# epruesse/metacov

Hardware: AMD Instinct MI355X
Metric: aligned bases/sec into per-position depth vector, 1/2/4/8 MI355X (higher is better)
Workload: dtype int32

## Files before the change

### metacov_amd/csrc/engine.hip

```cpp
#include <hip/hip_ext.h>
#include <hip/hip_runtime.h>

#include <algorithm>
#include <atomic>
#include <cmath>
#include <cstdlib>
#include <cstring>
#include <vector>

#include "../../include/metacov_amd.h"
#include "common.h"
#include "kernels.h"
#include "npstd.h"
#include "capmask.h"

#include <hipcub/hipcub.hpp>

using namespace mc;

#ifndef MC_PLAIN_TILES_PER_CHUNK
#define MC_PLAIN_TILES_PER_CHUNK 4
#endif
constexpr int kPlainTilesPerChunk = MC_PLAIN_TILES_PER_CHUNK;

// ... 1169 lines not shown
    const bool lds_hist = nbins <= kLdsBins;
    HIP_TRY(hipEventRecord(ctx->ev[6], s));
    int64_t launches = 0;
    for (int64_t r0 = 0; r0 < R; r0 += rb) {
        const int64_t nr = std::min(rb, R - r0);
        std::vector<int64_t> sg_gs, sg_ge, ntot(nr), nzx(nr);
        std::vector<int32_t> sg_reg;
        int64_t covered = 0;
        for (int64_t k = 0; k < nr; ++k) {
            const int64_t ext = ctx->extent[tid[r0 + k]];
            covered += std::min(end[r0 + k], ext) - std::min(start[r0 + k], ext);
        }
        int64_t seg = kSeg;
        while (seg > 16384 && covered / seg < 2048) seg >>= 1;
        for (int64_t k = 0; k < nr; ++k) {
            const int64_t r = r0 + k;
            const int32_t t = tid[r];
            const int64_t ext = ctx->extent[t];
            const int64_t a = std::min(start[r], ext), b = std::min(end[r], ext);
            ntot[k] = end[r] - start[r];
            nzx[k] = ntot[k] - (b - a);
            for (int64_t p = a; p < b; p += seg) {
                sg_gs.push_back(ctx->coff[t] + p);
                sg_ge.push_back(ctx->coff[t] + std::min(b, p + seg));
                sg_reg.push_back((int32_t)k);
            }
        }
        const int64_t nseg = (int64_t)sg_gs.size();
        const size_t o_gs = 0, o_ge = o_gs + stage_align(nseg * 8),
                     o_reg = o_ge + stage_align(nseg * 8), o_ntot = o_reg + stage_align(nseg * 4),
                     o_nzx = o_ntot + stage_align(nr * 8), o_rows = o_nzx + stage_align(nr * 8),
                     total = o_rows + (out_rows ? stage_align(nr * 8) : 0);
        HIP_TRY(ctx->k3_stage.reserve(total));
        unsigned char* h = ctx->k3_stage.host();
        std::memcpy(h + o_gs, sg_gs.data(), nseg * 8);
        std::memcpy(h + o_ge, sg_ge.data(), nseg * 8);
        std::memcpy(h + o_reg, sg_reg.data(), nseg * 4);
        std::memcpy(h + o_ntot, ntot.data(), nr * 8);
        std::memcpy(h + o_nzx, nzx.data(), nr * 8);
        if (out_rows) std::memcpy(h + o_rows, out_rows + r0, nr * 8);
        unsigned char* d = ctx->k3_stage.d.p;
        const int64_t* d_seg_gs = reinterpret_cast<const int64_t*>(d + o_gs);
        const int64_t* d_seg_ge = reinterpret_cast<const int64_t*>(d + o_ge);
        const int32_t* d_seg_reg = reinterpret_cast<const int32_t*>(d + o_reg);
        HIP_TRY(ctx->d_hist.reserve((size_t)round_up(nr * nbins, 4)));
        HIP_TRY(ctx->d_acc.reserve(nr));
        HIP_TRY(hipMemcpyAsync(d, h, total, hipMemcpyHostToDevice, s));
        {
            const int64_t hw = round_up(nr * nbins, 4);
            const int64_t work = std::max<int64_t>(hw / 4, nr);
            const unsigned g = (unsigned)std::min<int64_t>(4096, (work + kBlock - 1) / kBlock);
            hipLaunchKernelGGL(fused_init_kernel, dim3(std::max(g, 1u)), dim3(kBlock), 0, s,
                               ctx->d_hist.p, hw, (unsigned*)nullptr, ctx->d_acc.p, nr,
                               (const int64_t*)nullptr, (int64_t)0, (int64_t)1, (int64_t)0,
                               (int64_t*)nullptr, (unsigned*)nullptr, (int*)nullptr);
            HIP_TRY(hipGetLastError());
        }
        if (nseg) {
            if (lds_hist)
                hipLaunchKernelGGL(region_seg_kernel<true>, dim3((unsigned)nseg), dim3(kBlock),
                                   (size_t)round_up(nbins, 4) * 4, s, ctx->d_depth.p, d_seg_gs, d_seg_ge,
                                   d_seg_reg, nbins, ctx->d_hist.p, ctx->d_acc.p);
            else
                hipLaunchKernelGGL(region_seg_kernel<false>, dim3((unsigned)nseg), dim3(kBlock), 0,
                                   s, ctx->d_depth.p, d_seg_gs, d_seg_ge, d_seg_reg, nbins,
                                   ctx->d_hist.p, ctx->d_acc.p);
            HIP_TRY(hipGetLastError());
            ++launches;
        }
        hipLaunchKernelGGL(region_final_kernel, dim3((unsigned)nr), dim3(kBlock), 0, s,
                           ctx->d_hist.p, nbins, ctx->d_acc.p,
                           reinterpret_cast<const int64_t*>(d + o_ntot),
                           reinterpret_cast<const int64_t*>(d + o_nzx),
                           out_rows ? d_out_final : d_out_final + r0, (int*)nullptr, 1,
                           (const int32_t*)nullptr, (const unsigned*)nullptr, 1,
                           out_rows ? reinterpret_cast<const int64_t*>(d + o_rows) : nullptr);
        HIP_TRY(hipGetLastError());
        HIP_TRY(hipStreamSynchronize(s));
    }
    HIP_TRY(hipEventRecord(ctx->ev[7], s));
    ctx->t_stats = true;
    ctx->t.stats_launches += launches;
    return MC_OK;
}


struct FusedLayout {
    size_t gs, ge, id, base, ntot, nzx, brow, rtid, rfused, up, total;
};
static FusedLayout fused_layout(int64_t nf, int64_t R) {
    auto al = stage_align;
    FusedLayout L;
    L.gs = 0;
    L.ge = L.gs + al(nf * 8);
    L.id = L.ge + al(nf * 8);
    L.base = L.id + al(nf * 4);
    L.ntot = L.base + al(nf * 4);
    L.nzx = L.ntot + al(R * 8);
    L.brow = L.nzx + al(R * 8);
    L.rtid = L.brow + al(R * 4);
    L.rfused = L.rtid + al(R * 4);
    L.up = L.rfused + al(R * 4);
    L.total = L.up;
    return L;
}

constexpr int kRedo = 1;

static size_t fflag_ints(int64_t R) { return (size_t)round_up(R + 1, 2) + 2 * kDresWords; }
static unsigned long long* fflag_dres(int* base, int64_t R) {
    return reinterpret_cast<unsigned long long*>(base + round_up(R + 1, 2));
}

static int direct_verdict_sync(mc_ctx* ctx) {
    if (!ctx->direct || ctx->direct_checked) return MC_OK;
    unsigned long long* res = static_cast<unsigned long long*>(ctx->pin_io.h);
    HIP_TRY(hipMemcpyAsync(res, ctx->d_dres.p, kDresWords * 8, hipMemcpyDeviceToHost, ctx->stream));
    HIP_TRY(hipStreamSynchronize(ctx->stream));
    if (check_direct(ctx, res)) return MC_OK;
    direct_fallback(ctx, res);
    return kRedo;
}

#ifndef MC_DONE_MODE
#define MC_DONE_MODE 1
#endif
static int wait_event_spin(hipEvent_t ev) {
    for (;;) {
        const hipError_t e = hipEventQuery(ev);
        if (e == hipSuccess) return MC_OK;
        if (e != hipErrorNotReady) HIP_TRY(e);
        __builtin_ia32_pause();
    }
}

static int wait_stamp(mc_ctx* ctx, unsigned long long seq) {
    if (!ctx->stamp_ok) {
        HIP_TRY(hipStreamSynchronize(ctx->stream));
        return MC_OK;
    }
    for (unsigned k = 1;; ++k) {
        if (__atomic_load_n(ctx->h_done.h, __ATOMIC_ACQUIRE) >= seq) return MC_OK;
        __builtin_ia32_pause();
        if ((k & 1023) == 0) {
            const hipError_t e = hipStreamQuery(ctx->stream);
            if (e == hipSuccess) return MC_OK;
            if (e != hipErrorNotReady) HIP_TRY(e);
        }
    }
}

static int depth_stats_launch(mc_ctx* ctx, int64_t R, const int32_t* tid, const int64_t* start,
                              const int64_t* end, RegionOut* d_out, int64_t nf) {
    hipStream_t s = ctx->stream;
    const FusedLayout L = fused_layout(nf, R);
    const size_t o_gs = L.gs, o_ge = L.ge, o_id = L.id, o_base = L.base, o_ntot = L.ntot,
                 o_nzx = L.nzx, o_brow = L.brow;
    const K2Geom geo = k2_geom(ctx, true);
    HIP_TRY(ctx->d_fchunk.reserve(geo.n_chunks));
    HIP_TRY(ctx->d_flow.reserve(R));
    const int vals = fused_hist_vals(ctx->has_long);
    HIP_TRY(ctx->d_fhist.reserve((size_t)(R * vals)));
    HIP_TRY(ctx->h_fflag.reserve(fflag_ints(R)));
    const bool verdict = ctx->direct && !ctx->direct_checked;
    HIP_TRY(ctx->d_acc.reserve(R));
    unsigned char* d = ctx->fstage.d.p;
    const int64_t* d_fge = reinterpret_cast<const int64_t*>(d + o_ge);
    const bool clean = ctx->fused_clean && ctx->fused_clean_R == R && ctx->fcache.chunk_first;
    ctx->fused_clean = false;
    if (!clean) {
        const int64_t idx_chunks = ctx->fcache.chunk_first ? 0 : geo.n_chunks;
        const int64_t work = std::max<int64_t>({R * vals / 4, R, idx_chunks});
        const unsigned g = (unsigned)std::min<int64_t>(4096, (work + kBlock - 1) / kBlock);
        hipLaunchKernelGGL(fused_init_kernel, dim3(std::max(g, 1u)), dim3(kBlock), 0, s,
                           ctx->d_fhist.p, R * vals, ctx->d_flow.p, ctx->d_acc.p, R, d_fge, nf,
                           geo.chunk_w, idx_chunks, ctx->d_fchunk.p, ctx->d_queue.p,
                           ctx->d_maxdepth.p);
        HIP_TRY(hipGetLastError());
        ctx->fcache.chunk_first = true;
    } else if (ctx->check_clean) {
        HIP_TRY(ctx->d_check.reserve(1));
        HIP_TRY(hipMemsetAsync(ctx->d_check.p, 0, sizeof(unsigned long long), s));
        hipLaunchKernelGGL(fused_clean_check_kernel, dim3(1024), dim3(kBlock), 0, s, ctx->d_fhist.p, R * vals,
                           ctx->d_flow.p, ctx->d_acc.p, R, ctx->d_queue.p, ctx->d_maxdepth.p, ctx->d_check.p);
        HIP_TRY(hipGetLastError());
        unsigned long long bad = 0;
        HIP_TRY(hipMemcpyAsync(&bad, ctx->d_check.p, sizeof bad, hipMemcpyDeviceToHost, s));
        HIP_TRY(hipStreamSynchronize(s));
        MC_REQUIRE(bad == 0, MC_E_STATE, "fused buffers not initialised on a clean call (%llu words differ)", bad);
    }
    FusedRegions fr{nf,
                    ctx->d_fchunk.p,
                    reinterpret_cast<const int64_t*>(d + o_gs),
                    d_fge,
                    reinterpret_cast<const int32_t*>(d + o_id),
                    reinterpret_cast<const int32_t*>(d + o_base),
                    reinterpret_cast<const int32_t*>(d + L.rtid),
                    ctx->d_acc.p,
                    ctx->d_fhist.p,
                    ctx->d_flow.p};
    if (nf == 0) fr.n = 0;
    auto& T = ctx->ts[ctx->ts_cur];
    if (int rc = launch_depth(ctx, fr, T.e[1], T.e[2])) return rc;
    const unsigned long long seq = ++ctx->done_seq;
    unsigned long long* stamp = nullptr;
    if (ctx->stamp_ok) {
        if (!ctx->h_done.h) {
            if (ctx->h_done.reserve(1) != hipSuccess || ctx->d_kdone.reserve(1) != hipSuccess ||
                hipMemsetAsync(ctx->d_kdone.p, 0, sizeof(unsigned), s) != hipSuccess) {
                (void)hipGetLastError();
                ctx->stamp_ok = false;
            } else {
                __atomic_store_n(ctx->h_done.h, 0ull, __ATOMIC_RELEASE);
            }
        }
        if (ctx->stamp_ok && MC_DONE_MODE == 1) stamp = ctx->h_done.d;
    }
    const bool devfb = ctx->has_long || ctx->fb_recent;
    FbArgs F{};
    if (devfb) {
        if (!ctx->d_fb_cnt.p) {
            HIP_TRY(ctx->d_fb_hist.reserve((size_t)kFbSlots * kLdsBins));
            HIP_TRY(ctx->d_fb_acc.reserve(kFbSlots));
            HIP_TRY(ctx->d_fb_list.reserve(kFbSlots));
            HIP_TRY(ctx->d_fb_cnt.reserve(2));
            HIP_TRY(hipMemsetAsync(ctx->d_fb_cnt.p, 0, 8, s));
            hipLaunchKernelGGL(fused_init_kernel, dim3(1024), dim3(kBlock), 0, s, ctx->d_fb_hist.p,
                               (int64_t)kFbSlots * kLdsBins, (unsigned*)nullptr, ctx->d_fb_acc.p,
                               (int64_t)kFbSlots, (const int64_t*)nullptr, (int64_t)0, (int64_t)1, (int64_t)0,
                               (int64_t*)nullptr, (unsigned*)nullptr, (int*)nullptr);
            HIP_TRY(hipGetLastError());
        }
        F = FbArgs{ctx->d_depth.p,
                   reinterpret_cast<const int32_t*>(d + L.rfused),
                   reinterpret_cast<const int64_t*>(d + o_gs),
                   reinterpret_cast<const int64_t*>(d + o_ge),
                   reinterpret_cast<const int64_t*>(d + o_ntot),
                   reinterpret_cast<const int64_t*>(d + o_nzx),
                   ctx->h_fflag.d + R,
                   ctx->d_fb_list.p,
                   ctx->d_fb_cnt.p,
                   (int)(ctx->fb_calls & 1),
                   ctx->d_fb_hist.p,
                   ctx->d_fb_acc.p,
                   d_out};
        ctx->fb_calls += 1;
    }
    hipEvent_t k3_stop = MC_STEP_EVENTS && MC_EXT_EVENTS ? T.e[3] : nullptr;
#define MC_LAUNCH_K3B(V)                                                                           \
    hipExtLaunchKernelGGL(region_final_wave_kernel<V>, dim3((unsigned)((R + kWaves - 1) / kWaves)),     \
                          dim3(kBlock), 0u, s, nullptr, devfb ? nullptr : k3_stop, 0u,                   \
                          ctx->d_fhist.p, R, ctx->d_acc.p,                                              \
                       reinterpret_cast<const int64_t*>(d + o_ntot),                                \
                       reinterpret_cast<const int64_t*>(d + o_nzx), d_out, ctx->h_fflag.d,           \
                       reinterpret_cast<const int32_t*>(d + o_brow), ctx->d_flow.p,                 \
                       ctx->d_maxdepth.p, ctx->h_fflag.d + R, ctx->d_queue.p,                       \
                       verdict ? ctx->d_dres.p : nullptr, verdict ? fflag_dres(ctx->h_fflag.d, R) : nullptr, \
                       devfb ? F.cnt + F.parity : nullptr, devfb ? F.list : nullptr,                \
                       ctx->direct ? direct_window(ctx) : DirectWindow{},                          \
                       ctx->direct ? reinterpret_cast<const int32_t*>(d + L.rtid) : nullptr,           \
                       ctx->d_kdone.p, devfb ? nullptr : stamp, seq)
    if (vals == HistCfg<false>::kBins) MC_LAUNCH_K3B(HistCfg<false>::kBins);
    else MC_LAUNCH_K3B(HistCfg<true>::kBins);
#undef MC_LAUNCH_K3B
    HIP_TRY(hipGetLastError());
    if (devfb) {
        hipLaunchKernelGGL(fb_seg_kernel, dim3(1024), dim3(kBlock), (size_t)kLdsBins * 4, s, F);
        HIP_TRY(hipGetLastError());
        hipExtLaunchKernelGGL(fb_final_kernel, dim3(kFbSlots), dim3(kBlock), 0u, s, nullptr, k3_stop, 0u, F);
        HIP_TRY(hipGetLastError());
    }
    if (MC_STEP_EVENTS && !MC_EXT_EVENTS) HIP_TRY(hipEventRecord(T.e[3], s));
    if ((MC_DONE_MODE == 0 || (MC_DONE_MODE == 1 && devfb)) && ctx->stamp_ok && hipStreamWriteValue64(s, ctx->h_done.d, seq, 0) != hipSuccess) {
        (void)hipGetLastError();
        ctx->stamp_ok = false;
    }
    ctx->t_stats = false;
    ctx->t.stats_launches += 1;
    resolve_timings(ctx, false);
    if (int rc = MC_DONE_MODE == 2 ? wait_event_spin(T.e[3]) : wait_stamp(ctx, seq)) return rc;
    const int* flags = ctx->h_fflag.h;
    if (verdict && !check_direct(ctx, fflag_dres(ctx->h_fflag.h, R), true)) {
// ... 467 lines not shown
```

### metacov_amd/csrc/kernels.h

```cpp
#pragma once

#include <hip/hip_runtime.h>
#include <stdint.h>

namespace mc {

#ifndef MC_TILE_W
#define MC_TILE_W 4096
#endif
#ifndef MC_RING
#define MC_RING (2 * MC_TILE_W)
#endif
#ifndef MC_TILES_PER_CHUNK
#define MC_TILES_PER_CHUNK 8
#endif
#ifndef MC_PREFETCH
#define MC_PREFETCH 1
#endif
#ifndef MC_PREFETCH_STATS
#define MC_PREFETCH_STATS 1
#endif
#ifndef MC_APPLY_SHORT
#define MC_APPLY_SHORT 1
#endif
#ifndef MC_FAR_HALO
#define MC_FAR_HALO 1
#endif
#ifndef MC_FAR_HALO_MIN
#define MC_FAR_HALO_MIN 4096
#endif
#ifndef MC_DIRECT_ONE_CONTIG
#define MC_DIRECT_ONE_CONTIG 1
#endif
#ifndef MC_K2_WAVE_ADVANCE
#define MC_K2_WAVE_ADVANCE 0
#endif
#ifndef MC_FILL_WAVE_COUNTS
#define MC_FILL_WAVE_COUNTS 0
#endif
#ifndef MC_FILL_SORTED
#define MC_FILL_SORTED 0
#endif
#ifndef MC_DEFER_LONG
#define MC_DEFER_LONG 1
#endif
#ifndef MC_DEFER_DIRECT
#define MC_DEFER_DIRECT 0
#endif
#ifndef MC_NT_STORE
#define MC_NT_STORE 1
#endif
#ifndef MC_WAVES_PLAIN
#define MC_WAVES_PLAIN 0
#endif
#ifndef MC_WAVES_STATS
#define MC_WAVES_STATS 4
#endif
constexpr int kGposBits = 18;
constexpr unsigned kGposMask = (1u << kGposBits) - 1u;
constexpr int kGspanCap = (1 << (32 - kGposBits)) - 1;

constexpr int kBlock = 256;
constexpr int kWaves = kBlock / 64;
constexpr int kTileW = MC_TILE_W;
constexpr int kRing = MC_RING;
static_assert(kRing % 256 == 0 && kRing > kTileW, "ring must hold a tile plus a halo");

__device__ __forceinline__ int ring_slot(int rel) { return rel % kRing; }
constexpr int kTilesPerChunk = MC_TILES_PER_CHUNK;
#ifndef MC_TILES_PER_CHUNK_LONG
#define MC_TILES_PER_CHUNK_LONG 16
#endif
constexpr int kTilesPerChunkLong = MC_TILES_PER_CHUNK_LONG;
constexpr int kReadsPerThread = 4;
constexpr int kBatch = kBlock * kReadsPerThread;
#ifndef MC_K2_WAVES
#define MC_K2_WAVES 4
#endif
constexpr int kK2Waves = MC_K2_WAVES;
constexpr int kK2Block = 64 * kK2Waves;
constexpr int kK2Batch = kK2Block * kReadsPerThread;
constexpr int kPadBatch = kK2Batch > kBatch ? kK2Batch : kBatch;
static_assert(kK2Waves == 4 || kK2Waves == 8, "K2 workgroups of 4 or 8 waves");
constexpr int kLdsHeader = (4 + 2 * kK2Waves + 4 + 3) / 4 * 4 > 20 ? (4 + 2 * kK2Waves + 4 + 3) / 4 * 4 : 20;
constexpr int kSeg = 65536;
constexpr int kLdsBins = 16384;

typedef int i32x4 __attribute__((ext_vector_type(4)));

struct RegionAcc {
    unsigned long long sum;
    unsigned long long sumsq;
    int min;
    int max;
};


__device__ __forceinline__ int wave_incl_scan(int v, int lane) {
    (void)lane;
    v += __builtin_amdgcn_update_dpp(0, v, 0x111, 0xf, 0xf, false);
    v += __builtin_amdgcn_update_dpp(0, v, 0x112, 0xf, 0xf, false);
    v += __builtin_amdgcn_update_dpp(0, v, 0x114, 0xf, 0xf, false);
    v += __builtin_amdgcn_update_dpp(0, v, 0x118, 0xf, 0xf, false);
    v += __builtin_amdgcn_update_dpp(0, v, 0x142, 0xa, 0xf, false);
    v += __builtin_amdgcn_update_dpp(0, v, 0x143, 0xc, 0xf, false);
    return v;
}

__device__ __forceinline__ int wave_sum_i32(int v) {
// ... 421 lines not shown
#pragma unroll
        for (int w = 1; w < kWaves; ++w)
            v = threadIdx.x == 3 ? max(v, red[3][w]) : v + red[threadIdx.x][w];
        if (threadIdx.x == 3) atomicMax(&out[3], (unsigned long long)v);
        else if (v) atomicAdd(&out[threadIdx.x], (unsigned long long)v);
    }
}

constexpr int kProbeShift = 8;
constexpr int kNearHalo = 256;
constexpr int kFarHaloMin = MC_FAR_HALO_MIN;
constexpr int kProbeStride = 1 << kProbeShift;

enum : int {
    kDresBadSample = 0,
    kDresLongSample = 1,
    kDresFlags = 2,
    kDresBases = 3,
    kDresMaxSpan = 4,
    kDresSpanSum = 5,
    kDresSpanCnt = 6,
    kDresWords = 9
};
constexpr unsigned kDirectInvalid = 1;
constexpr unsigned kDirectUnfit = 2;

struct ProbeArgs {
    const int32_t* tid;
    const int32_t* pos;
    const int32_t* span;
    int64_t n;
    int32_t nc;
    const int64_t* coff;
    int lw;
    int short_max;
    int halo;
    int64_t n_base;
    int32_t* j0;
    int32_t* jh;
    int32_t* jn;
    int32_t* fsamp;
    unsigned long long* dres;
    unsigned long long gen;
};

struct DirectWindow {
    const int32_t* fsamp;
    const int64_t* len;
    const unsigned long long* dres;
    int parity;
    int win_below;
};

template <class WT>
__device__ __forceinline__ int direct_window_base(const WT& W, int parity, int t) {
    const long long ns = (long long)uload(W.fsamp, t + 1) - uload(W.fsamp, t);
    const unsigned long long ssum = uload(W.dres, kDresSpanSum + 2 * parity);
    const unsigned long long scnt = uload(W.dres, kDresSpanCnt + 2 * parity);
    if (ns <= 0 || scnt == 0) return 0;
    const double mean = (double)ssum / (double)scnt;
    const double bases = (double)ns * (double)kProbeStride * mean;
    const double ext = (double)uload(W.len, t);
    const double body = ext > 2.0 * mean ? ext - mean : ext;
    const double est = ext > 0 ? bases / body : 0.0;
    const long long b0 = llrint(est) - W.win_below;
    return b0 > 0 ? (int)b0 : 0;
}

__device__ __forceinline__ int64_t probe_key(const ProbeArgs& A, int t, int p) {
    const int ct = t < 0 ? 0 : t >= A.nc ? A.nc - 1 : t;
    const int64_t k = A.coff[ct] + (int64_t)(p < 0 ? 0 : p);
    return k;
}

__device__ __forceinline__ void probe_fill(int32_t* J, int64_t n_base, int lw, int64_t off, int64_t key,
                                           int64_t key_next, bool first, bool last, int32_t val) {
    int64_t k0 = first ? 0 : ((key + off) >> lw) + 1;
    int64_t k1 = last ? n_base : ((key_next + off) >> lw);
    if (k1 > n_base) k1 = n_base;
    if (first) {
        int64_t kz = (key + off) >> lw;
        if (kz > n_base) kz = n_base;
        for (int64_t k = 0; k <= kz; ++k) J[k] = 0;
        k0 = kz + 1;
    }
    for (int64_t k = k0; k <= k1; ++k) J[k] = val;
}

constexpr int kProbeSpanEvery = 4;
constexpr unsigned kProbeMeanBlocks = 64;

__global__ void __launch_bounds__(kBlock)
probe_kernel(ProbeArgs A) {
    const int64_t M = (A.n + kProbeStride - 1) >> kProbeShift;
    const int64_t j = (int64_t)blockIdx.x * kBlock + threadIdx.x;
    const int par = (int)(A.gen & 1);
    if (blockIdx.x == 0 && threadIdx.x >= kDresFlags && threadIdx.x <= kDresMaxSpan) A.dres[threadIdx.x] = 0;
    if (blockIdx.x == 0 && threadIdx.x < 2) A.dres[kDresSpanSum + 2 * (par ^ 1) + threadIdx.x] = 0;
    const bool sampled = j < M && (j % kProbeSpanEvery) == 0;
    const int s0 = sampled ? A.span[j << kProbeShift] : 0;
    const unsigned every = max(1u, gridDim.x / kProbeMeanBlocks);
    if (blockIdx.x % every == 0) {
        __shared__ long long red[2 * kWaves];
        const bool s_ok = sampled && s0 >= 0;
        const long long wsum = wave_sum64(s_ok ? (long long)s0 : 0);
        const long long wcnt = wave_sum64(s_ok ? 1 : 0);
        if ((threadIdx.x & 63) == 0) {
            red[threadIdx.x >> 6] = wsum;
            red[kWaves + (threadIdx.x >> 6)] = wcnt;
        }
        __syncthreads();
        if (threadIdx.x == 0) {
            long long ts = 0, tc = 0;
#pragma unroll
            for (int w = 0; w < kWaves; ++w) {
                ts += red[w];
                tc += red[kWaves + w];
            }
            if (tc) {
// ... 832 lines not shown
    __syncthreads();
    if (threadIdx.x == 0) {
        long long t = 0;
#pragma unroll
        for (int w = 0; w < kWaves; ++w) t += ws[w];
        part[blockIdx.x] = (unsigned long long)t;
    }
}

__global__ void __launch_bounds__(kBlock)
span_sum_final_kernel(const unsigned long long* __restrict__ part, int m, unsigned long long* __restrict__ out) {
    long long s = 0;
    for (int i = threadIdx.x; i < m; i += kBlock) s += (long long)part[i];
    s = wave_sum64(s);
    __shared__ long long ws[kWaves];
    if ((threadIdx.x & 63) == 0) ws[threadIdx.x >> 6] = s;
    __syncthreads();
    if (threadIdx.x == 0) {
        long long t = 0;
#pragma unroll
        for (int w = 0; w < kWaves; ++w) t += ws[w];
        *out = (unsigned long long)t;
    }
}

#ifndef MC_HIST_COPIES
#define MC_HIST_COPIES 2
#endif
#ifndef MC_HIST_BINS
#define MC_HIST_BINS (MC_HIST_COPIES == 1 ? 1024 : MC_HIST_COPIES == 2 ? 864 \
                      : MC_HIST_COPIES == 4 ? 480 : MC_HIST_COPIES == 8 ? 224 : 96)
#endif
#ifndef MC_HIST_COPIES_LONG
#define MC_HIST_COPIES_LONG MC_HIST_COPIES
#endif
#ifndef MC_HIST_BINS_LONG
#define MC_HIST_BINS_LONG (MC_HIST_COPIES_LONG == 1 ? 1728 : MC_HIST_BINS)
#endif
template <bool kLong>
struct HistCfg {
    static constexpr int kCopies = kLong ? MC_HIST_COPIES_LONG : MC_HIST_COPIES;
    static constexpr int kBins = kLong ? MC_HIST_BINS_LONG : MC_HIST_BINS;
    static constexpr int kPad = kCopies > 1 ? 32 / kCopies : 32;
    static constexpr int kStride = kBins + kPad;
    static constexpr int kLds = kCopies * kStride;
    static_assert(kBins % 32 == 0 && (kCopies & (kCopies - 1)) == 0 && kCopies <= 32,
                  "histogram bins: multiple of 32; copies: power of two");
};
constexpr int kHistBins = HistCfg<false>::kBins;
__host__ __device__ constexpr int fused_hist_vals(bool long_reads) {
    return long_reads ? HistCfg<true>::kBins : HistCfg<false>::kBins;
}

struct FusedRegions {
    int64_t n;
    const int64_t* chunk_first;
    const int64_t* gs;
    const int64_t* ge;
    const int32_t* id;
    const int32_t* base;
    const int32_t* rtid;
    RegionAcc* acc;
    unsigned* hist;
    unsigned* low;
};

struct OvLds {
    unsigned long long sum, sq;
    int vmin, vmax;
    unsigned cnt, low;
    unsigned pad[2];
};
constexpr int kOvRecs = 16;
static_assert(sizeof(OvLds) == 40, "record stride: 10 banks");
constexpr int kOvInts = kOvRecs * (int)sizeof(OvLds) / 4;

__device__ __forceinline__ void ov_reset(OvLds* ov) {
    ov->sum = ov->sq = 0;
    ov->vmin = 0x7fffffff;
    ov->vmax = 0;
    ov->cnt = ov->low = 0;
}

struct OvReg {
    unsigned cnt, low;
    unsigned long long sum, sq;
    int vmin, vmax;
};

__device__ __forceinline__ void ov_reg_reset(OvReg& r) {
    r.cnt = r.low = 0;
    r.sum = r.sq = 0;
    r.vmin = 0x7fffffff;
    r.vmax = 0;
}

__device__ __attribute__((noinline)) void ov_spill(OvLds* ov, unsigned cnt, unsigned low, unsigned long long sum,
                                                   unsigned long long sq, int mn, int mx) {
    if (cnt) {
        atomicAdd(&ov->cnt, cnt);
        if (low) atomicAdd(&ov->low, low);
        atomicAdd(&ov->sum, sum);
        atomicAdd(&ov->sq, sq);
        atomicMin(&ov->vmin, mn);
        atomicMax(&ov->vmax, mx);
    }
}

__device__ __forceinline__ void ov_reg_spill(OvReg& r, OvLds* ovf) {
    if (__any(r.cnt != 0)) {
        ov_spill(ovf + (threadIdx.x & (kOvRecs - 1)), r.cnt, r.low, r.sum, r.sq, r.vmin, r.vmax);
        ov_reg_reset(r);
    }
}

static_assert(kRing == 2 * kTileW, "the ring tail is one tile (short_max = kTileW)");

template <int kWinBins>
__device__ __forceinline__ void hist_int4(unsigned* h, int dummy, OvReg& ovr, int y0, int y1, int y2, int y3,
                                          int base) {
    const bool s1 = y1 != y0, s2 = y2 != y1, s3 = y3 != y2;
    const int l2 = s3 ? 1 : 2;
    const int l1 = s2 ? 1 : l2 + 1;
    const int l0 = s1 ? 1 : l1 + 1;
    constexpr unsigned kWin = (unsigned)kWinBins;
    const unsigned du = (unsigned)dummy;
    const unsigned d0 = (unsigned)(y0 - base), d1 = (unsigned)(y1 - base),
                   d2 = (unsigned)(y2 - base), d3 = (unsigned)(y3 - base);
    atomicAdd(&h[min(d0, du)], (unsigned)l0);
    atomicAdd(&h[s1 ? min(d1, du) : du], (unsigned)l1);
    atomicAdd(&h[s2 ? min(d2, du) : du], (unsigned)l2);
    atomicAdd(&h[s3 ? min(d3, du) : du], 1u);
    if (__builtin_expect(__any(max(max(d0, d1), max(d2, d3)) >= kWin), 0)) {
        const int y[4] = {y0, y1, y2, y3};
        const unsigned d[4] = {d0, d1, d2, d3};
#pragma unroll
        for (int k = 0; k < 4; ++k) {
            const bool o = (y[k] >= 0) & (d[k] >= kWin);
            const unsigned v = o ? (unsigned)y[k] : 0u;
            ovr.cnt += o ? 1u : 0u;
            ovr.low += (o & (y[k] < base)) ? 1u : 0u;
            ovr.sum += v;
            ovr.sq += (unsigned long long)v * v;
            ovr.vmin = min(ovr.vmin, o ? y[k] : 0x7fffffff);
            ovr.vmax = max(ovr.vmax, (int)v);
        }
    }
}

__device__ __forceinline__ void block_all2(int* words, int& flip, bool p0, bool p1, int wave, int lane,
                                           bool& all0, bool& all1) {
    const int v = (__all(p0) ? 1 : 0) | (__all(p1) ? 2 : 0);
    if (lane == 0) reinterpret_cast<unsigned char*>(words + 2 * flip)[wave] = (unsigned char)v;
    __syncthreads();
    if (kK2Waves == 4) {
        const int w = words[2 * flip];
        all0 = (w & 0x01010101) == 0x01010101;
        all1 = (w & 0x02020202) == 0x02020202;
    } else {
        const unsigned long long w = *reinterpret_cast<const unsigned long long*>(words + 2 * flip);
        all0 = (w & 0x0101010101010101ull) == 0x0101010101010101ull;
        all1 = (w & 0x0202020202020202ull) == 0x0202020202020202ull;
    }
    flip ^= 1;
}

struct EvBatch {
    int rel[4];
    unsigned pending;
};

__device__ __forceinline__ void load_events(EvBatch& e, const int32_t* __restrict__ ev, int64_t base,
                                            int64_t e_lo, int64_t e_hi) {
    const int64_t i0 = base + (int64_t)threadIdx.x * 4;
    e.pending = 0;
    if (i0 < e_hi && i0 + 4 > e_lo) {
        const i32x4 x = *reinterpret_cast<const i32x4*>(ev + i0);
        e.rel[0] = x.x;
        e.rel[1] = x.y;
        e.rel[2] = x.z;
        e.rel[3] = x.w;
#pragma unroll
        for (int k = 0; k < 4; ++k)
            if (i0 + k >= e_lo && i0 + k < e_hi) e.pending |= 1u << k;
    }
}

template <bool kBarriers, class HC, class RT>
__device__ __forceinline__ void flush_region(const RT& R, int id, unsigned* h, OvLds* ov) {
    if (kBarriers) __syncthreads();
    if (threadIdx.x < kOvRecs) {
        OvLds* o = ov + threadIdx.x;
        if (o->cnt) {
            if (o->low) atomicAdd(&R.low[id], o->low);
            atomicMin(&R.acc[id].min, o->vmin);
            atomicMax(&R.acc[id].max, o->vmax);
            atomicAdd(&R.acc[id].sum, o->sum);
            atomicAdd(&R.acc[id].sumsq, o->sq);
            ov_reset(o);
        }
    }
    unsigned* g = R.hist + (int64_t)id * HC::kBins;
    for (int k = threadIdx.x; k < HC::kBins; k += kK2Block) {
        unsigned cnt = 0;
#pragma unroll
        for (int c = 0; c < HC::kCopies; ++c) cnt += h[c * HC::kStride + k];
        if (cnt) {
            atomicAdd(&g[k], cnt);
#pragma unroll
            for (int c = 0; c < HC::kCopies; ++c) h[c * HC::kStride + k] = 0;
        }
    }
    if (kBarriers) __syncthreads();
}

__device__ __forceinline__ int take_chunk(unsigned* queue, int64_t n_chunks) {
    const unsigned t = atomicAdd(queue, 1u);
    return t < (unsigned)n_chunks ? (int)t : (int)n_chunks;
}

struct K2Consts {
    ReadArrays A;
    FusedRegions R;
    DirectArgs D;
};

template <bool kStats, bool kLong, bool kDirect>
__global__ void __launch_bounds__(kK2Block, kStats ? (MC_WAVES_STATS ? MC_WAVES_STATS : 1)
                                                 : (MC_WAVES_PLAIN ? MC_WAVES_PLAIN : 1))
depth_kernel(ReadArrays A, const K2Consts* __restrict__ K, int64_t n,
             const int64_t* __restrict__ coff, const int64_t* __restrict__ chunk_first,
             int cstride, int64_t n_chunks, int tiles_per_chunk, int short_max,
             const int64_t* __restrict__ tile_ev_off, const int32_t* __restrict__ tile_ev,
             const int* __restrict__ chunk_carry,
             int32_t* __restrict__ depth, unsigned* __restrict__ queue,
             int* __restrict__ max_depth, unsigned long long gen, int win_parity) {
    static_assert(!(kDirect && kLong), "the direct path has no long reads");
    const auto& KC = *(const __attribute__((address_space(4))) K2Consts*)K;
    const auto& R = KC.R;
    const auto& D = KC.D;
    extern __shared__ __attribute__((aligned(16))) int lds[];
    int* hdr = lds;
    int and_flip = 0;
    int* ring = lds + kLdsHeader;
    unsigned* hist = reinterpret_cast<unsigned*>(ring + kRing);
    using HC = HistCfg<kLong>;
    OvLds* ovf = reinterpret_cast<OvLds*>(hist + HC::kLds);
    const int lane = threadIdx.x & 63;
    unsigned* hist_lane = hist + (lane & (HC::kCopies - 1)) * HC::kStride;
    const int hist_dummy = HC::kBins + (lane / HC::kCopies) % HC::kPad;
    const int wave = __builtin_amdgcn_readfirstlane(threadIdx.x >> 6);
    const int64_t chunk_w = (int64_t)tiles_per_chunk * kTileW;
    constexpr int kWaveSpan = kTileW / kK2Waves;
    constexpr int kChunks = kWaveSpan / (64 * 4);
    constexpr bool kDefer = !kStats || (kLong && MC_DEFER_LONG) || (kDirect && MC_DEFER_DIRECT);
    constexpr bool kPf = kStats ? MC_PREFETCH_STATS : MC_PREFETCH;
    if (kDirect) {
        const unsigned long long f0 = uload(D.dres, kDresBadSample), f1 = uload(D.dres, kDresLongSample);
        if (f0 == gen || f1 == gen) return;
    }
    int my_max = 0;
    DirectAcc dacc;
    OvReg ovr;
    ov_reg_reset(ovr);
    if (kStats) {
        for (int k = threadIdx.x; k < HC::kLds; k += kK2Block) hist[k] = 0;
        if (threadIdx.x < kOvRecs) ov_reset(ovf + threadIdx.x);
    }

    constexpr bool kAhead = kStats && kLong;
    int ticket = 0;
    if (threadIdx.x == 0) hdr[0] = take_chunk(queue, n_chunks);
    const int ring_tail = (int)(((int64_t)tiles_per_chunk * kTileW) % kRing);
    for (int k = threadIdx.x * 4; k < kRing; k += kK2Block * 4)
        *reinterpret_cast<i32x4*>(ring + k) = i32x4{0, 0, 0, 0};
    for (;;) {
        __syncthreads();
        const int64_t c = (unsigned)__builtin_amdgcn_readfirstlane(hdr[0]);
        if (c >= n_chunks) break;
        if (kAhead && threadIdx.x == 0) ticket = take_chunk(queue, n_chunks);
        const int64_t b0 = c * cstride;
        int64_t cfirst, cend;
        DirectChunk dc{0, 0, 0, 0};
        int64_t far_lo = 0, far_hi = 0;
        if (kDirect) {
            const int64_t b1 = b0 + cstride;
            auto lower = [&](int64_t J) { return J <= 0 ? (int64_t)0 : min(n, ((J - 1) << kProbeShift) + 1); };
            auto upper = [&](int64_t J) { return J <= 0 ? (int64_t)0 : min(n, J << kProbeShift); };
            const bool last = c + 1 == n_chunks;
            dc.lo = c ? lower(uload(D.jh, b0)) : 0;
            dc.vlo = c ? lower(uload(D.j0, b0)) : 0;
            dc.hi = last ? n : upper(uload(D.j0, b1));
            dc.vhi = last ? n : lower(uload(D.j0, b1));
            dc.lo = min(dc.lo, dc.vlo);
            dc.hi = max(dc.hi, dc.vhi);
            if (MC_FAR_HALO && c) {
                const int64_t fh = min(max(lower(uload(D.jn, b0)), dc.lo), dc.vlo);
                if (fh - dc.lo >= kFarHaloMin) {
                    far_lo = dc.lo;
                    far_hi = fh;
                    dc.lo = fh;
                }
            }
            cfirst = dc.lo;
            cend = dc.hi;
        } else {
            cfirst = b0 ? (int64_t)min((uint64_t)uload(chunk_first, 2 * b0),
                                       (uint64_t)uload(chunk_first, 2 * b0 - 1)) : 0;
            cend = uload(chunk_first, 2 * (c + 1) * cstride - 1);
        }
        const int64_t C0 = c * chunk_w;
        int64_t rcur = 0, r_gs = 0, r_ge = 0;
        int r_base = 0, r_id = 0;
        if (kStats) {
            rcur = uload(R.chunk_first, c);
            if (rcur < R.n) {
                r_gs = uload(R.gs, rcur);
                r_ge = uload(R.ge, rcur);
                r_id = uload(R.id, rcur);
                r_base = kDirect ? direct_window_base(D.win, win_parity, uload(R.rtid, r_id)) : uload(R.base, rcur);
            }
        }
        int64_t base = cfirst & ~(int64_t)(kReadsPerThread - 1);
        bool more = base < cend;
        ReadBatch b;
        RawBatch<kDirect> nxt;
        b.pending = 0;
        auto finish = [&](const RawBatch<kDirect>& r, int64_t at) {
            if constexpr (kDirect)
                finish_batch_direct(b, r, at, C0, chunk_w, dc, coff, D, short_max, dacc);
            else
                finish_batch(b, r, at, cend, C0, cfirst);
        };
        RawBatch<kDirect> r0;
        if (more) {
            issue_raw<kDirect>(r0, base, A, cend);
            if (kPf && base + kK2Batch < cend) issue_raw<kDirect>(nxt, base + kK2Batch, A, cend);
        }
        if (kDirect && MC_FAR_HALO && far_hi > far_lo) far_halo(A, D, coff, far_lo, far_hi, C0, short_max, ring);
        if (more) finish(r0, base);
        int carry = kLong ? uload(chunk_carry, c) : 0;
        EvBatch eb;
        eb.pending = 0;
        int64_t ev_lo = 0, ev_hi = 0, ev_base = 0;
        bool ev_more = false;
        if (kLong) {
            ev_lo = uload(tile_ev_off, c * tiles_per_chunk);
            ev_hi = uload(tile_ev_off, (c + 1) * tiles_per_chunk);
            ev_base = ev_lo & ~(int64_t)3;
            ev_more = ev_base < ev_hi;
            if (ev_more) load_events(eb, tile_ev, ev_base, ev_lo, ev_hi);
        }
        i32x4 v[kChunks];
        int64_t pend_T0 = -1;
        auto store_tile = [&](int64_t tile0) {
            int32_t* dst = depth + tile0 + wave * kWaveSpan + lane * 4;
#pragma unroll
            for (int j = 0; j < kChunks; ++j) {
                if (MC_NT_STORE)
                    __builtin_nontemporal_store(v[j], reinterpret_cast<i32x4*>(dst + j * 256));
                else
                    *reinterpret_cast<i32x4*>(dst + j * 256) = v[j];
            }
        };
        for (int t = 0; t < tiles_per_chunk; ++t) {
            const int64_t T0 = C0 + (int64_t)t * kTileW;
            const int64_t Tend = T0 + kTileW;
            const int tend_rel = (t + 1) * kTileW;
            for (;;) {
                if (kLong) {
#pragma unroll
                    for (int k = 0; k < 4; ++k)
                        if (((eb.pending >> k) & 1u) && eb.rel[k] < tend_rel) {
                            atomicAdd(&ring[ring_slot(eb.rel[k])], -1);
                            eb.pending &= ~(1u << k);
                        }
                }
                if (MC_APPLY_SHORT && !kLong) {
                    unsigned done = 0;
#pragma unroll
                    for (int k = 0; k < kReadsPerThread; ++k) {
                        const bool go = ((b.pending >> k) & 1u) && b.rs[k] < tend_rel;
                        done |= go ? 1u << k : 0u;
                        const int s = b.rs[k] > 0 ? b.rs[k] : 0, e = b.rs[k] + b.sp[k];
                        if (MC_APPLY_SHORT == 2) {
                            const bool ap = go && e > s;
                            if (__ballot(ap)) {
                                atomicAdd(&ring[ring_slot(s)], ap ? 1 : 0);
                                atomicAdd(&ring[ring_slot(e)], ap ? -1 : 0);
                            }
                        } else if (go && e > s) {
                            atomicAdd(&ring[ring_slot(s)], 1);
                            atomicAdd(&ring[ring_slot(e)], -1);
                        }
                    }
                    b.pending &= ~done;
                } else
#pragma unroll
                for (int k = 0; k < kReadsPerThread; ++k) {
                    if (((b.pending >> k) & 1u) && b.rs[k] < tend_rel) {
                        const int rs = b.rs[k], sp = b.sp[k];
                        if (sp <= short_max) {
                            const int s = rs > 0 ? rs : 0;
                            const int e = rs + sp;
                            if (e > s) {
// ... 50 lines not shown
                const int incl = wave_incl_scan(x.w, lane);
                const int excl = incl - x.w + wave_total;
                x += excl;
                v[j] = x;
                wave_total += __builtin_amdgcn_readlane(incl, 63);
            }
            if (lane == 0) hdr[4 + wave] = wave_total;
            __syncthreads();
            int off = carry, tile_total = 0;
#pragma unroll
            for (int w = 0; w < kK2Waves; ++w) {
                const int tw = hdr[4 + w];
                if (w < wave) off += tw;
                tile_total += tw;
            }
            carry += tile_total;
#pragma unroll
            for (int j = 0; j < kChunks; ++j) {
                i32x4 x = v[j] + off;
                v[j] = x;
                my_max = max(my_max, max(max(x.x, x.y), max(x.z, x.w)));
            }
            if (kDefer) {
                pend_T0 = T0;
            } else {
                store_tile(T0);
            }
            if (kStats) {
                while (rcur < R.n && r_gs < Tend) {
                    const int64_t rgs = r_gs, rge = r_ge;
                    const int lo = (int)((rgs > T0 ? rgs : T0) - T0);
                    const int hi = (int)((rge < Tend ? rge : Tend) - T0);
                    const bool full = lo == 0 && hi == kTileW;
#pragma unroll
                    for (int j = 0; j < kChunks; ++j) {
                        int y0 = v[j].x, y1 = v[j].y, y2 = v[j].z, y3 = v[j].w;
                        if (!full) {
                            const int q0 = wave * kWaveSpan + j * 256 + lane * 4;
                            y0 = (q0 >= lo && q0 < hi) ? y0 : -1;
                            y1 = (q0 + 1 >= lo && q0 + 1 < hi) ? y1 : -1;
                            y2 = (q0 + 2 >= lo && q0 + 2 < hi) ? y2 : -1;
                            y3 = (q0 + 3 >= lo && q0 + 3 < hi) ? y3 : -1;
                        }
                        hist_int4<HC::kBins>(hist_lane, hist_dummy, ovr, y0, y1, y2, y3, r_base);
                    }
                    if (rge <= Tend) {
                        ov_reg_spill(ovr, ovf);
                        flush_region<true, HC>(R, r_id, hist, ovf);
                        ++rcur;
                        if (rcur < R.n) {
                            r_gs = uload(R.gs, rcur);
                            r_ge = uload(R.ge, rcur);
                            r_id = uload(R.id, rcur);
                            r_base = kDirect ? direct_window_base(D.win, win_parity, uload(R.rtid, r_id))
                                             : uload(R.base, rcur);
                        }
                    } else {
                        break;
                    }
                }
            }
        }
        if (kDefer && pend_T0 >= 0) store_tile(pend_T0);
        if (kStats) ov_reg_spill(ovr, ovf);
        __syncthreads();
        if (kStats) {
            if (rcur < R.n && r_gs < C0 + chunk_w) flush_region<false, HC>(R, r_id, hist, ovf);
        }
        if (threadIdx.x == 0) hdr[0] = kAhead ? ticket : take_chunk(queue, n_chunks);
        for (int k = threadIdx.x * 4; k < kTileW; k += kK2Block * 4)
            *reinterpret_cast<i32x4*>(ring + ring_tail + k) = i32x4{0, 0, 0, 0};
    }
    my_max = wave_max(my_max);
    if (lane == 0) hdr[4 + kK2Waves + wave] = my_max;
    __syncthreads();
    if (threadIdx.x == 0) {
        int m = 0;
#pragma unroll
        for (int w = 0; w < kK2Waves; ++w) m = max(m, hdr[4 + kK2Waves + w]);
        if (m > 0) atomicMax(max_depth, m);
    }
    if (kDirect) direct_flush(dacc, D, ring);
}


__global__ void __launch_bounds__(kBlock)
fused_init_kernel(unsigned* __restrict__ hist, int64_t hist_words, unsigned* __restrict__ low,
                  RegionAcc* __restrict__ acc, int64_t R, const int64_t* __restrict__ fge,
                  int64_t nf, int64_t chunk_w, int64_t n_chunks, int64_t* __restrict__ chunk_first,
                  unsigned* __restrict__ queue, int* __restrict__ max_depth) {
    if (blockIdx.x == 0 && threadIdx.x < 8) {
        if (queue) queue[threadIdx.x] = 0;
        if (max_depth && threadIdx.x < 4) max_depth[threadIdx.x] = 0;
    }
    const int64_t stride = (int64_t)gridDim.x * kBlock;
    const int64_t i0 = blockIdx.x * (int64_t)kBlock + threadIdx.x;
    for (int64_t q = i0; q * 4 < hist_words; q += stride)
        *reinterpret_cast<i32x4*>(hist + q * 4) = i32x4{0, 0, 0, 0};
    for (int64_t r = i0; r < R; r += stride) {
        if (low) low[r] = 0;
        acc[r].sum = 0;
        acc[r].sumsq = 0;
        acc[r].min = 0x7fffffff;
        acc[r].max = 0;
    }
    for (int64_t c = i0; c < n_chunks; c += stride) {
        const int64_t C0 = c * chunk_w;
        int64_t lo = 0, hi = nf;
        while (lo < hi) {
            const int64_t mid = (lo + hi) >> 1;
            if (fge[mid] <= C0) lo = mid + 1;
            else hi = mid;
        }
        chunk_first[c] = lo;
    }
}

__global__ void __launch_bounds__(kBlock)
fused_clean_check_kernel(const unsigned* __restrict__ hist, int64_t hist_words, const unsigned* __restrict__ low,
                         const RegionAcc* __restrict__ acc, int64_t R, const unsigned* __restrict__ queue,
                         const int* __restrict__ max_depth, unsigned long long* __restrict__ bad) {
    unsigned long long n = 0;
    if (blockIdx.x == 0 && threadIdx.x < 8) {
        if (queue && queue[threadIdx.x] != 0) ++n;
        if (max_depth && threadIdx.x < 4 && max_depth[threadIdx.x] != 0) ++n;
    }
    const int64_t stride = (int64_t)gridDim.x * kBlock;
    const int64_t i0 = blockIdx.x * (int64_t)kBlock + threadIdx.x;
    for (int64_t q = i0; q < hist_words; q += stride) n += hist[q] != 0;
    for (int64_t r = i0; r < R; r += stride) {
        n += (low && low[r] != 0) ? 1 : 0;
        n += (acc[r].sum != 0) + (acc[r].sumsq != 0) + (acc[r].min != 0x7fffffff) + (acc[r].max != 0);
    }
    n = (unsigned long long)wave_sum64((long long)n);
    if ((threadIdx.x & 63) == 0 && n) atomicAdd(bad, n);
}

template <bool kLdsHist>
__global__ void __launch_bounds__(kBlock)
region_seg_kernel(const int32_t* __restrict__ depth, const int64_t* __restrict__ seg_gs,
                  const int64_t* __restrict__ seg_ge, const int32_t* __restrict__ seg_reg,
                  int nbins, unsigned* __restrict__ hist, RegionAcc* __restrict__ acc) {
    extern __shared__ __attribute__((aligned(16))) unsigned h[];
    const int64_t sgi = blockIdx.x;
    const int64_t gs = seg_gs[sgi], ge = seg_ge[sgi];
    const int r = seg_reg[sgi];
    unsigned* ghist = hist + (int64_t)r * nbins;
    unsigned* hh = kLdsHist ? h : ghist;
    if (kLdsHist) {
        for (int k = threadIdx.x * 4; k < nbins; k += kBlock * 4)
            *reinterpret_cast<i32x4*>(h + k) = i32x4{0, 0, 0, 0};
        __syncthreads();
    }
    constexpr int kU = 4;
    int vmax = 0;
    unsigned vmin = 0xffffffffu;
    const int64_t a4 = gs & ~(int64_t)3;
    for (int64_t p0 = a4 + (int64_t)threadIdx.x * 4; p0 < ge; p0 += (int64_t)kBlock * 4 * kU) {
        i32x4 x[kU];
#pragma unroll
        for (int u = 0; u < kU; ++u) {
            const int64_t p = p0 + (int64_t)u * kBlock * 4;
            x[u] = p < ge ? __builtin_nontemporal_load(reinterpret_cast<const i32x4*>(depth + p))
                          : i32x4{-1, -1, -1, -1};
        }
#pragma unroll
        for (int u = 0; u < kU; ++u) {
// ... 486 lines not shown
```

Measured before the change: 14340 billion.

## Precompute per-chunk region descriptors and hoist chunk-start scalar loads ahead of batch work

The init kernel now writes a 32-byte descriptor per chunk (first region index, gs, ge, id, rtid) so the per-chunk kernel can fetch it with one scalar load instead of a chain of dependent loads. Window-base inputs, halo indices and event offsets are loaded early and evaluated after the first read batch is issued, to overlap their latency with that batch. The low and count overlap counters are packed into one 32-bit word, and the next-chunk ticket grab moves later in the chunk. This adds descriptor memory and complexity, and the packed 16-bit counters could overflow if a thread accumulates many overlaps before spilling.

New measurement: 14500 billion (median of 5 runs). 1.01x the previous value.

```diff
diff --git a/metacov_amd/csrc/engine.hip b/metacov_amd/csrc/engine.hip
--- a/metacov_amd/csrc/engine.hip
+++ b/metacov_amd/csrc/engine.hip
@@ -1245,7 +1245,8 @@
             const unsigned g = (unsigned)std::min<int64_t>(4096, (work + kBlock - 1) / kBlock);
             hipLaunchKernelGGL(fused_init_kernel, dim3(std::max(g, 1u)), dim3(kBlock), 0, s,
                                ctx->d_hist.p, hw, (unsigned*)nullptr, ctx->d_acc.p, nr,
-                               (const int64_t*)nullptr, (int64_t)0, (int64_t)1, (int64_t)0,
+                               (const int64_t*)nullptr, (const int64_t*)nullptr, (const int32_t*)nullptr,
+                               (const int32_t*)nullptr, (int64_t)0, (int64_t)1, (int64_t)0,
                                (int64_t*)nullptr, (unsigned*)nullptr, (int*)nullptr);
             HIP_TRY(hipGetLastError());
         }
@@ -1350,7 +1351,7 @@
     const size_t o_gs = L.gs, o_ge = L.ge, o_id = L.id, o_base = L.base, o_ntot = L.ntot,
                  o_nzx = L.nzx, o_brow = L.brow;
     const K2Geom geo = k2_geom(ctx, true);
-    HIP_TRY(ctx->d_fchunk.reserve(geo.n_chunks));
+    HIP_TRY(ctx->d_fchunk.reserve(geo.n_chunks * kFchunkWords));
     HIP_TRY(ctx->d_flow.reserve(R));
     const int vals = fused_hist_vals(ctx->has_long);
     HIP_TRY(ctx->d_fhist.reserve((size_t)(R * vals)));
@@ -1366,7 +1367,10 @@
         const int64_t work = std::max<int64_t>({R * vals / 4, R, idx_chunks});
         const unsigned g = (unsigned)std::min<int64_t>(4096, (work + kBlock - 1) / kBlock);
         hipLaunchKernelGGL(fused_init_kernel, dim3(std::max(g, 1u)), dim3(kBlock), 0, s,
-                           ctx->d_fhist.p, R * vals, ctx->d_flow.p, ctx->d_acc.p, R, d_fge, nf,
+                           ctx->d_fhist.p, R * vals, ctx->d_flow.p, ctx->d_acc.p, R,
+                           reinterpret_cast<const int64_t*>(d + o_gs), d_fge,
+                           reinterpret_cast<const int32_t*>(d + o_id),
+                           reinterpret_cast<const int32_t*>(d + L.rtid), nf,
                            geo.chunk_w, idx_chunks, ctx->d_fchunk.p, ctx->d_queue.p,
                            ctx->d_maxdepth.p);
         HIP_TRY(hipGetLastError());
@@ -1420,7 +1424,8 @@
             HIP_TRY(hipMemsetAsync(ctx->d_fb_cnt.p, 0, 8, s));
             hipLaunchKernelGGL(fused_init_kernel, dim3(1024), dim3(kBlock), 0, s, ctx->d_fb_hist.p,
                                (int64_t)kFbSlots * kLdsBins, (unsigned*)nullptr, ctx->d_fb_acc.p,
-                               (int64_t)kFbSlots, (const int64_t*)nullptr, (int64_t)0, (int64_t)1, (int64_t)0,
+                               (int64_t)kFbSlots, (const int64_t*)nullptr, (const int64_t*)nullptr,
+                               (const int32_t*)nullptr, (const int32_t*)nullptr, (int64_t)0, (int64_t)1, (int64_t)0,
                                (int64_t*)nullptr, (unsigned*)nullptr, (int*)nullptr);
             HIP_TRY(hipGetLastError());
         }
diff --git a/metacov_amd/csrc/kernels.h b/metacov_amd/csrc/kernels.h
--- a/metacov_amd/csrc/kernels.h
+++ b/metacov_amd/csrc/kernels.h
@@ -55,6 +55,24 @@
 #endif
 #ifndef MC_WAVES_STATS
 #define MC_WAVES_STATS 4
+#endif
+#ifndef MC_CHUNK_AHEAD
+#define MC_CHUNK_AHEAD 0
+#endif
+#ifndef MC_CHUNK_AHEAD_TAIL
+#define MC_CHUNK_AHEAD_TAIL 2
+#endif
+#ifndef MC_OV_PACK
+#define MC_OV_PACK 1
+#endif
+#ifndef MC_ZERO_OFF_OPAQUE
+#define MC_ZERO_OFF_OPAQUE MC_CHUNK_AHEAD
+#endif
+#ifndef MC_CHUNK_DESC
+#define MC_CHUNK_DESC 1
+#endif
+#ifndef MC_CHUNK_LOADS_FIRST
+#define MC_CHUNK_LOADS_FIRST 1
 #endif
 constexpr int kGposBits = 18;
 constexpr unsigned kGposMask = (1u << kGposBits) - 1u;
@@ -582,19 +600,38 @@
     int win_below;
 };
 
+struct WindowIn {
+    long long ns;
+    unsigned long long ssum, scnt;
+    long long len;
+    int win_below;
+};
+
+template <class WT>
+__device__ __forceinline__ WindowIn direct_window_load(const WT& W, int parity, int t) {
+    WindowIn in;
+    in.ns = (long long)uload(W.fsamp, t + 1) - uload(W.fsamp, t);
+    in.ssum = uload(W.dres, kDresSpanSum + 2 * parity);
+    in.scnt = uload(W.dres, kDresSpanCnt + 2 * parity);
+    in.len = uload(W.len, t);
+    in.win_below = W.win_below;
+    return in;
+}
+
+__device__ __forceinline__ int direct_window_eval(const WindowIn& in) {
+    if (in.ns <= 0 || in.scnt == 0) return 0;
+    const double mean = (double)in.ssum / (double)in.scnt;
+    const double bases = (double)in.ns * (double)kProbeStride * mean;
+    const double ext = (double)in.len;
+    const double body = ext > 2.0 * mean ? ext - mean : ext;
+    const double est = ext > 0 ? bases / body : 0.0;
+    const long long b0 = llrint(est) - in.win_below;
+    return b0 > 0 ? (int)b0 : 0;
+}
+
 template <class WT>
 __device__ __forceinline__ int direct_window_base(const WT& W, int parity, int t) {
-    const long long ns = (long long)uload(W.fsamp, t + 1) - uload(W.fsamp, t);
-    const unsigned long long ssum = uload(W.dres, kDresSpanSum + 2 * parity);
-    const unsigned long long scnt = uload(W.dres, kDresSpanCnt + 2 * parity);
-    if (ns <= 0 || scnt == 0) return 0;
-    const double mean = (double)ssum / (double)scnt;
-    const double bases = (double)ns * (double)kProbeStride * mean;
-    const double ext = (double)uload(W.len, t);
-    const double body = ext > 2.0 * mean ? ext - mean : ext;
-    const double est = ext > 0 ? bases / body : 0.0;
-    const long long b0 = llrint(est) - W.win_below;
-    return b0 > 0 ? (int)b0 : 0;
+    return direct_window_eval(direct_window_load(W, parity, t));
 }
 
 __device__ __forceinline__ int64_t probe_key(const ProbeArgs& A, int t, int p) {
@@ -1533,6 +1570,15 @@
     return long_reads ? HistCfg<true>::kBins : HistCfg<false>::kBins;
 }
 
+struct alignas(16) ChunkDesc {
+    int64_t rcur;
+    int64_t gs, ge;
+    int32_t id;
+    int32_t rtid;
+};
+static_assert(sizeof(ChunkDesc) == 32, "one s_load_dwordx8");
+constexpr int kFchunkWords = MC_CHUNK_DESC ? (int)(sizeof(ChunkDesc) / sizeof(int64_t)) : 1;
+
 struct FusedRegions {
     int64_t n;
     const int64_t* chunk_first;
@@ -1564,13 +1610,14 @@
 }
 
 struct OvReg {
-    unsigned cnt, low;
+    unsigned cl;
+    unsigned low;
     unsigned long long sum, sq;
     int vmin, vmax;
 };
 
 __device__ __forceinline__ void ov_reg_reset(OvReg& r) {
-    r.cnt = r.low = 0;
+    r.cl = r.low = 0;
     r.sum = r.sq = 0;
     r.vmin = 0x7fffffff;
     r.vmax = 0;
@@ -1589,8 +1636,9 @@
 }
 
 __device__ __forceinline__ void ov_reg_spill(OvReg& r, OvLds* ovf) {
-    if (__any(r.cnt != 0)) {
-        ov_spill(ovf + (threadIdx.x & (kOvRecs - 1)), r.cnt, r.low, r.sum, r.sq, r.vmin, r.vmax);
+    if (__any(r.cl != 0)) {
+        ov_spill(ovf + (threadIdx.x & (kOvRecs - 1)), MC_OV_PACK ? r.cl & 0xffffu : r.cl,
+                 MC_OV_PACK ? r.cl >> 16 : r.low, r.sum, r.sq, r.vmin, r.vmax);
         ov_reg_reset(r);
     }
 }
@@ -1619,8 +1667,12 @@
         for (int k = 0; k < 4; ++k) {
             const bool o = (y[k] >= 0) & (d[k] >= kWin);
             const unsigned v = o ? (unsigned)y[k] : 0u;
-            ovr.cnt += o ? 1u : 0u;
-            ovr.low += (o & (y[k] < base)) ? 1u : 0u;
+            if (MC_OV_PACK) {
+                ovr.cl += (o ? 1u : 0u) + ((o & (y[k] < base)) ? 0x10000u : 0u);
+            } else {
+                ovr.cl += o ? 1u : 0u;
+                ovr.low += (o & (y[k] < base)) ? 1u : 0u;
+            }
             ovr.sum += v;
             ovr.sq += (unsigned long long)v * v;
             ovr.vmin = min(ovr.vmin, o ? y[k] : 0x7fffffff);
@@ -1699,6 +1751,13 @@
     const unsigned t = atomicAdd(queue, 1u);
     return t < (unsigned)n_chunks ? (int)t : (int)n_chunks;
 }
+
+__device__ __forceinline__ unsigned take_chunk_later(unsigned* queue) {
+    unsigned z, one;
+    asm volatile("v_mov_b32 %0, 0\n\tv_mov_b32 %1, 1" : "=&v"(z), "=v"(one));
+    return atomicAdd(queue + z, one);
+}
+constexpr unsigned kNoTicket = 0xffffffffu;
 
 struct K2Consts {
     ReadArrays A;
@@ -1749,8 +1808,11 @@
         if (threadIdx.x < kOvRecs) ov_reset(ovf + threadIdx.x);
     }
 
-    constexpr bool kAhead = kStats && kLong;
-    int ticket = 0;
+    constexpr bool kAhead = MC_CHUNK_AHEAD || (kStats && kLong);
+    const int64_t ahead_end =
+        MC_CHUNK_AHEAD ? n_chunks - (int64_t)MC_CHUNK_AHEAD_TAIL * (int64_t)gridDim.x : n_chunks;
+    unsigned ticket = kNoTicket;
+    auto window_base = [&](int t) { return direct_window_base(D.win, win_parity, t); };
     if (threadIdx.x == 0) hdr[0] = take_chunk(queue, n_chunks);
     const int ring_tail = (int)(((int64_t)tiles_per_chunk * kTileW) % kRing);
     for (int k = threadIdx.x * 4; k < kRing; k += kK2Block * 4)
@@ -1759,7 +1821,9 @@
         __syncthreads();
         const int64_t c = (unsigned)__builtin_amdgcn_readfirstlane(hdr[0]);
         if (c >= n_chunks) break;
-        if (kAhead && threadIdx.x == 0) ticket = take_chunk(queue, n_chunks);
+        const bool ahead = kAhead && c < ahead_end;
+        ticket = kNoTicket;
+        if (!MC_CHUNK_LOADS_FIRST && ahead && threadIdx.x == 0) ticket = take_chunk_later(queue);
         const int64_t b0 = c * cstride;
         int64_t cfirst, cend;
         DirectChunk dc{0, 0, 0, 0};
@@ -1769,14 +1833,25 @@
             auto lower = [&](int64_t J) { return J <= 0 ? (int64_t)0 : min(n, ((J - 1) << kProbeShift) + 1); };
             auto upper = [&](int64_t J) { return J <= 0 ? (int64_t)0 : min(n, J << kProbeShift); };
             const bool last = c + 1 == n_chunks;
-            dc.lo = c ? lower(uload(D.jh, b0)) : 0;
-            dc.vlo = c ? lower(uload(D.j0, b0)) : 0;
-            dc.hi = last ? n : upper(uload(D.j0, b1));
-            dc.vhi = last ? n : lower(uload(D.j0, b1));
+            int jh_0 = 0, j0_0 = 0, j0_1 = 0, jn_0 = 0;
+            if (MC_CHUNK_LOADS_FIRST) {
+                jh_0 = uload(D.jh, b0);
+                j0_0 = uload(D.j0, b0);
+                j0_1 = uload(D.j0, b1);
+                if (MC_FAR_HALO) jn_0 = uload(D.jn, b0);
+                asm volatile("" : "+s"(jh_0), "+s"(j0_0), "+s"(j0_1), "+s"(jn_0));
+            }
+            auto J = [&](const int32_t* p, int64_t at, int pre) {
+                return MC_CHUNK_LOADS_FIRST ? (int64_t)pre : (int64_t)uload(p, at);
+            };
+            dc.lo = c ? lower(J(D.jh, b0, jh_0)) : 0;
+            dc.vlo = c ? lower(J(D.j0, b0, j0_0)) : 0;
+            dc.hi = last ? n : upper(J(D.j0, b1, j0_1));
+            dc.vhi = last ? n : lower(J(D.j0, b1, j0_1));
             dc.lo = min(dc.lo, dc.vlo);
             dc.hi = max(dc.hi, dc.vhi);
             if (MC_FAR_HALO && c) {
-                const int64_t fh = min(max(lower(uload(D.jn, b0)), dc.lo), dc.vlo);
+                const int64_t fh = min(max(lower(J(D.jn, b0, jn_0)), dc.lo), dc.vlo);
                 if (fh - dc.lo >= kFarHaloMin) {
                     far_lo = dc.lo;
                     far_hi = fh;
@@ -1793,15 +1868,38 @@
         const int64_t C0 = c * chunk_w;
         int64_t rcur = 0, r_gs = 0, r_ge = 0;
         int r_base = 0, r_id = 0;
-        if (kStats) {
-            rcur = uload(R.chunk_first, c);
-            if (rcur < R.n) {
-                r_gs = uload(R.gs, rcur);
-                r_ge = uload(R.ge, rcur);
-                r_id = uload(R.id, rcur);
-                r_base = kDirect ? direct_window_base(D.win, win_parity, uload(R.rtid, r_id)) : uload(R.base, rcur);
-            }
-        }
+        WindowIn win_in{0, 0, 0, 0, 0};
+        bool win_open = false;
+        auto first_region = [&]() {
+            if (!kStats) return;
+            if (MC_CHUNK_DESC) {
+                const auto& cd = ((const __attribute__((address_space(4))) ChunkDesc*)R.chunk_first)[c];
+                rcur = cd.rcur;
+                r_gs = cd.gs;
+                r_ge = cd.ge;
+                r_id = cd.id;
+                const int r_tid = cd.rtid;
+                if (rcur < R.n) {
+                    if (kDirect && MC_CHUNK_LOADS_FIRST) {
+                        win_in = direct_window_load(D.win, win_parity, r_tid);
+                        asm volatile("" : "+s"(win_in.ns), "+s"(win_in.ssum), "+s"(win_in.scnt), "+s"(win_in.len),
+                                          "+s"(win_in.win_below));
+                        win_open = true;
+                    } else {
+                        r_base = kDirect ? window_base(r_tid) : uload(R.base, rcur);
+                    }
+                }
+            } else {
+                rcur = uload(R.chunk_first, c);
+                if (rcur < R.n) {
+                    r_gs = uload(R.gs, rcur);
+                    r_ge = uload(R.ge, rcur);
+                    r_id = uload(R.id, rcur);
+                    r_base = kDirect ? window_base(uload(R.rtid, r_id)) : uload(R.base, rcur);
+                }
+            }
+        };
+        if (!MC_CHUNK_LOADS_FIRST) first_region();
         int64_t base = cfirst & ~(int64_t)(kReadsPerThread - 1);
         bool more = base < cend;
         ReadBatch b;
@@ -1813,25 +1911,34 @@
             else
                 finish_batch(b, r, at, cend, C0, cfirst);
         };
-        RawBatch<kDirect> r0;
-        if (more) {
-            issue_raw<kDirect>(r0, base, A, cend);
-            if (kPf && base + kK2Batch < cend) issue_raw<kDirect>(nxt, base + kK2Batch, A, cend);
-        }
-        if (kDirect && MC_FAR_HALO && far_hi > far_lo) far_halo(A, D, coff, far_lo, far_hi, C0, short_max, ring);
-        if (more) finish(r0, base);
-        int carry = kLong ? uload(chunk_carry, c) : 0;
+        int carry = 0;
         EvBatch eb;
         eb.pending = 0;
         int64_t ev_lo = 0, ev_hi = 0, ev_base = 0;
         bool ev_more = false;
-        if (kLong) {
+        auto first_events = [&]() {
+            if (!kLong) return;
+            carry = uload(chunk_carry, c);
             ev_lo = uload(tile_ev_off, c * tiles_per_chunk);
             ev_hi = uload(tile_ev_off, (c + 1) * tiles_per_chunk);
             ev_base = ev_lo & ~(int64_t)3;
             ev_more = ev_base < ev_hi;
             if (ev_more) load_events(eb, tile_ev, ev_base, ev_lo, ev_hi);
-        }
+        };
+        RawBatch<kDirect> r0;
+        if (more) {
+            issue_raw<kDirect>(r0, base, A, cend);
+            if (kPf && base + kK2Batch < cend) issue_raw<kDirect>(nxt, base + kK2Batch, A, cend);
+        }
+        if (MC_CHUNK_LOADS_FIRST) {
+            first_region();
+            first_events();
+        }
+        if (kDirect && MC_FAR_HALO && far_hi > far_lo) far_halo(A, D, coff, far_lo, far_hi, C0, short_max, ring);
+        if (more) finish(r0, base);
+        if (win_open) r_base = direct_window_eval(win_in);
+        if (!MC_CHUNK_LOADS_FIRST) first_events();
+        if (MC_CHUNK_LOADS_FIRST && ahead && threadIdx.x == 0) ticket = take_chunk_later(queue);
         i32x4 v[kChunks];
         int64_t pend_T0 = -1;
         auto store_tile = [&](int64_t tile0) {
@@ -1988,8 +2095,7 @@
                             r_gs = uload(R.gs, rcur);
                             r_ge = uload(R.ge, rcur);
                             r_id = uload(R.id, rcur);
-                            r_base = kDirect ? direct_window_base(D.win, win_parity, uload(R.rtid, r_id))
-                                             : uload(R.base, rcur);
+                            r_base = kDirect ? window_base(uload(R.rtid, r_id)) : uload(R.base, rcur);
                         }
                     } else {
                         break;
@@ -2003,8 +2109,11 @@
         if (kStats) {
             if (rcur < R.n && r_gs < C0 + chunk_w) flush_region<false, HC>(R, r_id, hist, ovf);
         }
-        if (threadIdx.x == 0) hdr[0] = kAhead ? ticket : take_chunk(queue, n_chunks);
-        for (int k = threadIdx.x * 4; k < kTileW; k += kK2Block * 4)
+        if (threadIdx.x == 0)
+            hdr[0] = ticket != kNoTicket ? (int)min((uint64_t)ticket, (uint64_t)n_chunks) : take_chunk(queue, n_chunks);
+        int zero_off = (int)threadIdx.x * 4;
+        if (MC_ZERO_OFF_OPAQUE) asm volatile("" : "+v"(zero_off));
+        for (int k = zero_off; k < kTileW; k += kK2Block * 4)
             *reinterpret_cast<i32x4*>(ring + ring_tail + k) = i32x4{0, 0, 0, 0};
     }
     my_max = wave_max(my_max);
@@ -2022,7 +2131,9 @@
 
 __global__ void __launch_bounds__(kBlock)
 fused_init_kernel(unsigned* __restrict__ hist, int64_t hist_words, unsigned* __restrict__ low,
-                  RegionAcc* __restrict__ acc, int64_t R, const int64_t* __restrict__ fge,
+                  RegionAcc* __restrict__ acc, int64_t R, const int64_t* __restrict__ fgs,
+                  const int64_t* __restrict__ fge, const int32_t* __restrict__ fid,
+                  const int32_t* __restrict__ rtid,
                   int64_t nf, int64_t chunk_w, int64_t n_chunks, int64_t* __restrict__ chunk_first,
                   unsigned* __restrict__ queue, int* __restrict__ max_depth) {
     if (blockIdx.x == 0 && threadIdx.x < 8) {
@@ -2048,7 +2159,18 @@
             if (fge[mid] <= C0) lo = mid + 1;
             else hi = mid;
         }
-        chunk_first[c] = lo;
+        if (MC_CHUNK_DESC) {
+            ChunkDesc cd{lo, 0, 0, 0, 0};
+            if (lo < nf) {
+                cd.gs = fgs[lo];
+                cd.ge = fge[lo];
+                cd.id = fid[lo];
+                cd.rtid = rtid[cd.id];
+            }
+            reinterpret_cast<ChunkDesc*>(chunk_first)[c] = cd;
+        } else {
+            chunk_first[c] = lo;
+        }
     }
 }
 
```
